# DreamScene-Project/DreamScene

Hardware: AMD Instinct MI355X
Metric: fwd+bwd views/s @1024x1024, 500000 Gaussians (higher is better)
Workload: dtype f32

## Files before the change

### dreamscene_amd/csrc/radix_sort.h

```cpp
#pragma once
#include "gsr_common.h"
#include <type_traits>

namespace {

constexpr int kSortThreads = 256;
constexpr int kItemsLarge = 16;
constexpr int kItemsSmall = 4;
constexpr int kRadixBits = 8;
constexpr int kRadix = 1 << kRadixBits;

template <typename T>
__device__ __forceinline__ T* batch_ptr(T* p, size_t bstride) {
  typedef typename std::conditional<std::is_const<T>::value, const char, char>::type B;
  return p ? reinterpret_cast<T*>(reinterpret_cast<B*>(p) + (size_t)blockIdx.y * bstride) : p;
}
#define GSR_LDS_ORDER() asm volatile("" ::: "memory")

__device__ __forceinline__ uint64_t eff_count(const uint64_t* n_dev, uint64_t cap) {
  if (!n_dev) return cap;
  const uint64_t n = *n_dev;
  return n < cap ? n : cap;
}

// ... 183 lines not shown
    if (is_valid(it)) {
      const uint32_t d = (key[it] >> shift) & (kRadix - 1);
      const uint32_t pos = wh[wave][d] + rank[it];
      keys_out[pos] = key[it];
      vals_out[pos] = val[it];
    }
  }
}

#ifndef GSR_OS_ITEMS_SMALL
#define GSR_OS_ITEMS_SMALL 16
#endif
constexpr int kOsItemsSmall = GSR_OS_ITEMS_SMALL;
constexpr int kOsMaxPasses = 4;
#ifndef GSR_OS_HIST_TILE
#define GSR_OS_HIST_TILE 2048
#endif
constexpr uint32_t kOsHistTile = GSR_OS_HIST_TILE;
constexpr uint32_t kOsTableOff = kOsMaxPasses * kRadix + 16;
constexpr uint32_t kOsSkipFlag = kOsMaxPasses * kRadix + 8;
constexpr uint32_t kOsEarlyN = kOsMaxPasses * kRadix + 10;
constexpr uint64_t kOsMaxN = 1ull << 28;

typedef __attribute__((address_space(1))) uint32_t gsr_gu32;
__device__ __forceinline__ gsr_gu32* gsr_global(uint32_t* p) { return (gsr_gu32*)(uintptr_t)p; }

__host__ __device__ inline uint32_t os_tiles(uint64_t n, int items) {
  const uint64_t t = (uint64_t)kSortThreads * items;
  return (uint32_t)((n + t - 1) / t);
}
__host__ inline size_t os_state_words(uint64_t n, int items) { return (size_t)kOsTableOff + (size_t)kRadix * os_tiles(n, items); }

template <bool DROP>
__global__ void __launch_bounds__(kSortThreads)
k_os_hist(const uint32_t* __restrict__ keys, const uint64_t* __restrict__ n_dev, uint64_t cap, int passes,
          uint32_t* __restrict__ os, size_t bstride, const uint32_t* __restrict__ wrect) {
  keys = batch_ptr(keys, bstride); n_dev = batch_ptr(n_dev, bstride); os = batch_ptr(os, bstride);
  wrect = batch_ptr(wrect, bstride);
  __shared__ uint32_t h[kOsMaxPasses][kRadix];
  __shared__ uint32_t wsum[kSortThreads / 64];
  const int tid = threadIdx.x, lane = tid & 63;
  const uint64_t n = eff_count(n_dev, cap);
  const uint64_t base = (uint64_t)blockIdx.x * kOsHistTile;
  if (base >= n) return;
#pragma unroll
  for (int p = 0; p < kOsMaxPasses; ++p) h[p][tid] = 0;
  __syncthreads();
  constexpr int kPer = kOsHistTile / kSortThreads;
  uint32_t kk[kPer];
  uint32_t weight = 0;
#pragma unroll
  for (int it = 0; it < kPer; ++it) {
    const uint64_t e = base + (uint64_t)(it * kSortThreads + tid);
    kk[it] = e < n ? keys[e] : 0xFFFFFFFFu;
    if (wrect && e < n && (!DROP || kk[it] != 0xFFFFFFFFu)) {
      const uint32_t r = wrect[e];
      weight += (((r >> 16) & 255u) + 1u) * ((r >> 24) + 1u);
    }
  }
  if (wrect) {
#pragma unroll
    for (int o = 32; o > 0; o >>= 1) weight += (uint32_t)__shfl_xor((int)weight, o, 64);
    if (lane == 0) wsum[tid >> 6] = weight;
  }
#pragma unroll
  for (int it = 0; it < kPer; ++it) {
    const uint64_t e = base + (uint64_t)(it * kSortThreads + tid);
    const bool valid = (e < n) && (!DROP || kk[it] != 0xFFFFFFFFu);
    const unsigned long long vm = __ballot(valid);
    if (vm == 0ull) continue;
    const uint32_t k = kk[it];
    if (valid) {
      atomicAdd(&h[0][k & (kRadix - 1)], 1u);
      if (passes > 1) atomicAdd(&h[1][(k >> kRadixBits) & (kRadix - 1)], 1u);
    }
    if (passes > 2) {
      const int first = __ffsll((long long)vm) - 1;
      const uint32_t hi = k >> (2 * kRadixBits), hi0 = (uint32_t)__shfl((int)hi, first, 64);
      if (__ballot(valid && hi != hi0) == 0ull) {
        if (lane == first) {
          atomicAdd(&h[2][hi0 & (kRadix - 1)], (uint32_t)__popcll(vm));
          if (passes > 3) atomicAdd(&h[3][hi0 >> kRadixBits], (uint32_t)__popcll(vm));
        }
      } else if (valid) {
        atomicAdd(&h[2][hi & (kRadix - 1)], 1u);
        if (passes > 3) atomicAdd(&h[3][hi >> kRadixBits], 1u);
      }
    }
  }
  __syncthreads();
  for (int p = 0; p < passes; ++p) {
    const uint32_t c = h[p][tid];
    if (c) atomicAdd(&os[p * kRadix + tid], c);
  }
  if (wrect && tid == 0) {
    const uint64_t w = ((uint64_t)wsum[0] + wsum[1]) + ((uint64_t)wsum[2] + wsum[3]);
    if (w) atomicAdd(reinterpret_cast<unsigned long long*>(os + kOsEarlyN), (unsigned long long)w);
  }
}

#ifndef GSR_OS_WINDOW
#define GSR_OS_WINDOW 16
#endif
constexpr int kOsWindow = GSR_OS_WINDOW;
__device__ __forceinline__ uint32_t os_look_back(gsr_gu32* table, uint32_t tile, int col, uint32_t tagA, uint32_t tagI) {
  uint32_t excl = 0;
  int p = (int)tile - 1;
  for (;;) {
    uint32_t w[kOsWindow];
#pragma unroll
    for (int j = 0; j < kOsWindow; ++j)
      w[j] = (p - j >= 0) ? __hip_atomic_load(table + (size_t)(p - j) * kRadix + col, __ATOMIC_RELAXED, __HIP_MEMORY_SCOPE_AGENT)
                          : 0u;
    bool done = false, stalled = false;
#pragma unroll
    for (int j = 0; j < kOsWindow; ++j) {
      if (done || stalled) continue;
      const uint32_t tag = w[j] & 0xF0000000u;
      if (tag == tagI) { excl += w[j] & 0x0FFFFFFFu; done = true; }
      else if (tag == tagA) { excl += w[j] & 0x0FFFFFFFu; --p; }
      else stalled = true;
    }
    if (done) return excl;
    if (stalled) __builtin_amdgcn_s_sleep(1);
  }
}

#ifdef GSR_OS_TRACE
__device__ unsigned long long* g_os_trace = nullptr;
#define GSR_OS_STAMP(k) do { if (threadIdx.x == 0 && g_os_trace) \
    g_os_trace[(((size_t)pass * 4 + blockIdx.y) * 4096 + blockIdx.x) * 8 + (k)] = wall_clock64(); } while (0)
#else
#define GSR_OS_STAMP(k) do { } while (0)
#endif

template <bool IOTA, int ITEMS, bool DROP>
__global__ void __launch_bounds__(kSortThreads)
k_os_pass(const uint32_t* __restrict__ keys_in, const uint32_t* __restrict__ vals_in, uint32_t* __restrict__ keys_out,
          uint32_t* __restrict__ vals_out, const uint64_t* __restrict__ n_dev, uint64_t cap, int pass,
          uint32_t* __restrict__ os, uint64_t* __restrict__ n_out, size_t bstride, const int may_skip,
          uint64_t* __restrict__ early_out) {
  keys_in = batch_ptr(keys_in, bstride); vals_in = batch_ptr(vals_in, bstride);
  keys_out = batch_ptr(keys_out, bstride); vals_out = batch_ptr(vals_out, bstride);
  n_dev = batch_ptr(n_dev, bstride); os = batch_ptr(os, bstride); n_out = batch_ptr(n_out, bstride);
  constexpr uint32_t T = kSortThreads * ITEMS;
  __shared__ uint32_t wh[4][kRadix];
  __shared__ uint32_t gbase[kRadix];
  __shared__ uint32_t skey[T], sval[T];
  __shared__ uint32_t wtot[4];
  __shared__ uint32_t s_tile, s_ntile;
  const int tid = threadIdx.x, lane = tid & 63, wave = tid >> 6;
  const int shift = pass * kRadixBits;
  const uint64_t n = eff_count(n_dev, cap);
  if constexpr (!DROP) {
    const uint32_t x = os[pass * kRadix + tid];
    if (__syncthreads_or((uint64_t)x == n && n > 0)) {
      if (may_skip) {
        if (blockIdx.x == 0 && tid == 0) os[kOsSkipFlag] = 1u;
        return;
      }
#pragma unroll
      for (int it = 0; it < ITEMS; ++it) {
        const uint64_t e = sort_index<ITEMS>(blockIdx.x, wave, it, lane);
        if (e < n) {
          keys_out[e] = keys_in[e];
          vals_out[e] = IOTA ? (uint32_t)e : vals_in[e];
        }
      }
      return;
    }
  }
  GSR_OS_STAMP(0);
  if (tid == 0) s_tile = atomicAdd(&os[kOsMaxPasses * kRadix + pass], 1u);
#pragma unroll
  for (int w = 0; w < 4; ++w) wh[w][tid] = 0;
  __syncthreads();
  const uint32_t tile = s_tile;
  if (early_out && tile == 0 && tid == 0)
    __hip_atomic_store(early_out + blockIdx.y, *reinterpret_cast<const uint64_t*>(os + kOsEarlyN), __ATOMIC_RELAXED,
                       __HIP_MEMORY_SCOPE_SYSTEM);
  if ((uint64_t)tile * T >= n) return;
  uint32_t dbase;
  {
    const uint32_t x = os[pass * kRadix + tid];
    uint32_t inc = x;
#pragma unroll
    for (int o = 1; o < 64; o <<= 1) {
      const uint32_t t = (uint32_t)__shfl_up((int)inc, o, 64);
      if (lane >= o) inc += t;
    }
    if (lane == 63) wtot[wave] = inc;
    __syncthreads();
    uint32_t woff = 0;
    for (int w = 0; w < wave; ++w) woff += wtot[w];
    dbase = woff + inc - x;
    if (DROP && n_out && tile == 0 && tid == kSortThreads - 1) *n_out = (uint64_t)(woff + inc);
  }
  GSR_OS_STAMP(1);
#ifdef GSR_OS_TRACE
  if (threadIdx.x == 0 && g_os_trace) g_os_trace[(((size_t)pass * 4 + blockIdx.y) * 4096 + blockIdx.x) * 8 + 7] = tile;
#endif
  uint32_t* mywh = wh[wave];
  uint32_t key[ITEMS], val[ITEMS], rank[ITEMS];
  const unsigned long long lt = (1ull << lane) - 1ull;
#pragma unroll
  for (int it = 0; it < ITEMS; ++it) {
    const uint64_t e = sort_index<ITEMS>(tile, wave, it, lane);
    const bool valid = e < n;
    key[it] = valid ? keys_in[e] : 0xFFFFFFFFu;
    val[it] = IOTA ? (uint32_t)e : (valid ? vals_in[e] : 0u);
  }
  const auto is_valid = [&](int it) {
    const uint64_t e = sort_index<ITEMS>(tile, wave, it, lane);
    return (e < n) && (!DROP || key[it] != 0xFFFFFFFFu);
  };
#pragma unroll
  for (int it = 0; it < ITEMS; ++it) {
    const bool valid = is_valid(it);
    const uint32_t d = (key[it] >> shift) & (kRadix - 1);
    const unsigned long long m = match_digit(d, valid);
    const int leader = __ffsll((long long)m) - 1;
    uint32_t old = 0;
    if (valid && lane == leader) {
      old = mywh[d];
      mywh[d] = old + (uint32_t)__popcll(m);
    }
    old = (uint32_t)__shfl((int)old, valid ? leader : lane, 64);
    rank[it] = old + (uint32_t)__popcll(m & lt);
    GSR_LDS_ORDER();
  }
  __syncthreads();
  GSR_OS_STAMP(2);
  uint32_t cnt;
  {
    uint32_t run = 0;
#pragma unroll
    for (int w = 0; w < 4; ++w) {
      const uint32_t c = wh[w][tid];
      wh[w][tid] = run;
      run += c;
    }
    cnt = run;
  }
  gsr_gu32* table = gsr_global(os + kOsTableOff);
  const uint32_t tagA = (uint32_t)(2 * pass + 1) << 28, tagI = (uint32_t)(2 * pass + 2) << 28;
  uint32_t excl = 0;
  if (tile == 0) {
    __hip_atomic_store(table + tid, tagI | cnt, __ATOMIC_RELAXED, __HIP_MEMORY_SCOPE_AGENT);
  } else {
    __hip_atomic_store(table + (size_t)tile * kRadix + tid, tagA | cnt, __ATOMIC_RELAXED, __HIP_MEMORY_SCOPE_AGENT);
    excl = os_look_back(table, tile, tid, tagA, tagI);
    __hip_atomic_store(table + (size_t)tile * kRadix + tid, tagI | (excl + cnt), __ATOMIC_RELAXED, __HIP_MEMORY_SCOPE_AGENT);
  }
  GSR_OS_STAMP(3);
  uint32_t lstart;
  {
    uint32_t inc = cnt;
#pragma unroll
    for (int o = 1; o < 64; o <<= 1) {
      const uint32_t t = (uint32_t)__shfl_up((int)inc, o, 64);
      if (lane >= o) inc += t;
    }
    __syncthreads();
    if (lane == 63) wtot[wave] = inc;
    __syncthreads();
    uint32_t woff = 0;
    for (int w = 0; w < wave; ++w) woff += wtot[w];
    lstart = woff + inc - cnt;
    if (tid == kSortThreads - 1) s_ntile = woff + inc;
  }
#pragma unroll
  for (int w = 0; w < 4; ++w) wh[w][tid] += lstart;
  gbase[tid] = dbase + excl - lstart;
  __syncthreads();
#pragma unroll
  for (int it = 0; it < ITEMS; ++it) {
    if (is_valid(it)) {
      const uint32_t d = (key[it] >> shift) & (kRadix - 1);
      const uint32_t lp = wh[wave][d] + rank[it];
      skey[lp] = key[it];
      sval[lp] = val[it];
    }
  }
  __syncthreads();
  GSR_OS_STAMP(4);
  const uint32_t ntile = s_ntile;
  for (uint32_t i = tid; i < ntile; i += kSortThreads) {
    const uint32_t k = skey[i];
    const uint32_t pos = gbase[(k >> shift) & (kRadix - 1)] + i;
    keys_out[pos] = k;
    vals_out[pos] = sval[i];
  }
  GSR_OS_STAMP(5);
}

__host__ inline size_t align256(size_t x) { return (x + 255) & ~(size_t)255; }

uint32_t sort_blocks(uint64_t n, int items) {
  const uint64_t t = (uint64_t)kSortThreads * items;
  return (uint32_t)((n + t - 1) / t);
}

__host__ inline size_t sort_hist_bytes(uint64_t n, int items_legacy, int items_os) {
  const size_t legacy = (size_t)kRadix * sort_blocks(n, items_legacy) * 4;
  const size_t os = os_state_words(n, items_os) * 4;
  return align256(legacy > os ? legacy : os);
}

template <int ITEMS>
int radix_sort_u32_legacy(uint32_t* k0, uint32_t* v0, uint32_t* k1, uint32_t* v1, const uint64_t* n_dev, uint64_t cap,
                          int bits, bool iota, uint64_t* n_compact, uint32_t* hist, uint32_t* totals, hipStream_t stream,
                          int batch = 1, size_t bstride = 0);

template <int ITEMS, int OS_ITEMS>
int radix_sort_u32(uint32_t* k0, uint32_t* v0, uint32_t* k1, uint32_t* v1, const uint64_t* n_dev, uint64_t cap,
                   int bits, bool iota, uint64_t* n_compact, uint32_t* hist, uint32_t* totals, hipStream_t stream,
                   int batch = 1, size_t bstride = 0, bool state_cleared = false, bool last_pass_may_skip = false,
                   const uint32_t* early_rects = nullptr, uint64_t* early_out = nullptr) {
  const int passes = (bits + kRadixBits - 1) / kRadixBits;
  if (cap >= kOsMaxN || passes > kOsMaxPasses)
    return radix_sort_u32_legacy<ITEMS>(k0, v0, k1, v1, n_dev, cap, bits, iota, n_compact, hist, totals, stream, batch, bstride);
  const uint32_t ntile = os_tiles(cap, OS_ITEMS), nhist = (uint32_t)((cap + kOsHistTile - 1) / kOsHistTile);
  const dim3 grid(ntile, (uint32_t)batch), grid_h(nhist ? nhist : 1, (uint32_t)batch);
  if (!state_cleared &&
      gsr_zero_async(hist, os_state_words(cap, OS_ITEMS) * 4, stream, bstride, (uint32_t)batch) != hipSuccess) return passes & 1;
  const bool drop = iota && n_compact;
  if (!drop) { early_rects = nullptr; early_out = nullptr; }
  if (!early_out) early_rects = nullptr;
  if (drop)
    hipLaunchKernelGGL((k_os_hist<true>), grid_h, dim3(kSortThreads), 0, stream, k0, n_dev, cap, passes, hist, bstride,
                       early_rects);
  else
    hipLaunchKernelGGL((k_os_hist<false>), grid_h, dim3(kSortThreads), 0, stream, k0, n_dev, cap, passes, hist, bstride,
                       (const uint32_t*)nullptr);
  uint32_t *ka = k0, *va = v0, *kb = k1, *vb = v1;
  for (int p = 0; p < passes; ++p) {
    if (p == 0 && drop) {
      hipLaunchKernelGGL((k_os_pass<true, OS_ITEMS, true>), grid, dim3(kSortThreads), 0, stream, ka, va, kb, vb, n_dev, cap, p,
                         hist, n_compact, bstride, 0, early_rects ? early_out : (uint64_t*)nullptr);
      n_dev = n_compact;
    } else if (p == 0 && iota) {
      hipLaunchKernelGGL((k_os_pass<true, OS_ITEMS, false>), grid, dim3(kSortThreads), 0, stream, ka, va, kb, vb, n_dev, cap, p,
                         hist, (uint64_t*)nullptr, bstride, 0, (uint64_t*)nullptr);
    } else {
      hipLaunchKernelGGL((k_os_pass<false, OS_ITEMS, false>), grid, dim3(kSortThreads), 0, stream, ka, va, kb, vb, n_dev, cap, p,
                         hist, (uint64_t*)nullptr, bstride, (last_pass_may_skip && p == passes - 1 && p > 0) ? 1 : 0,
                         (uint64_t*)nullptr);
    }
    uint32_t* t = ka; ka = kb; kb = t;
    t = va; va = vb; vb = t;
  }
  return passes & 1;
}

template <int ITEMS>
int radix_sort_u32_legacy(uint32_t* k0, uint32_t* v0, uint32_t* k1, uint32_t* v1, const uint64_t* n_dev, uint64_t cap,
                   int bits, bool iota, uint64_t* n_compact, uint32_t* hist, uint32_t* totals, hipStream_t stream,
                   int batch, size_t bstride) {
  const uint32_t nblk = sort_blocks(cap, ITEMS);
  const int passes = (bits + kRadixBits - 1) / kRadixBits;
  const dim3 grid(nblk, (uint32_t)batch), grid_scan(kRadix, (uint32_t)batch);
  uint32_t *ka = k0, *va = v0, *kb = k1, *vb = v1;
  for (int p = 0; p < passes; ++p) {
// ... 29 lines not shown
```

### dreamscene_amd/csrc/render_bwd.hip

```cpp
#include "gsr_render.h"

namespace {

struct WorkBwdViews {
  const uint32_t* tile_depth[GSR_MAX_BATCH_VIEWS];
  uint32_t* items[GSR_MAX_BATCH_VIEWS];
  uint32_t items_cap[GSR_MAX_BATCH_VIEWS];
  uint32_t seg_len[GSR_MAX_BATCH_VIEWS];
};

__global__ void __launch_bounds__(1024)
k_work_order_bwd(const uint32_t n_tiles, const WorkBwdViews wv) {
  const uint32_t* __restrict__ tile_depth = wv.tile_depth[blockIdx.x];
  uint32_t* __restrict__ items = wv.items[blockIdx.x];
  const uint32_t items_cap = wv.items_cap[blockIdx.x];
  const uint32_t kb = wv.seg_len[blockIdx.x];
  __shared__ uint32_t cnt[32], cur[32];
  const int tid = threadIdx.x;
  if (tid < 32) cnt[tid] = 0;
  __syncthreads();
  for (uint32_t t = tid; t < n_tiles; t += 1024) {
    const uint32_t d = tile_depth[t];
    if (d == 0) continue;
    const uint32_t full = d / kb, tail = d % kb;
    for (uint32_t sgi = 0; sgi < full; ++sgi) atomicAdd(&cnt[15u - min(15u, (d - kb * sgi - 1u) >> 8)], 1u);
    if (tail) atomicAdd(&cnt[16u + 15u - ((tail - 1u) * 16u) / kb], 1u);
  }
  __syncthreads();
  if (tid == 0) {
    uint32_t run = 0;
    for (int b = 0; b < 32; ++b) { cur[b] = run; run += cnt[b]; }
    items[0] = min(run, items_cap);
  }
  __syncthreads();
  for (uint32_t t = tid; t < n_tiles; t += 1024) {
    const uint32_t d = tile_depth[t];
    if (d == 0) continue;
    const uint32_t full = d / kb, tail = d % kb;
    for (uint32_t sgi = 0; sgi < full; ++sgi) {
      const uint32_t i = atomicAdd(&cur[15u - min(15u, (d - kb * sgi - 1u) >> 8)], 1u);
      if (i < items_cap) { items[2 + 2 * i] = t; items[3 + 2 * i] = sgi; }
    }
    if (tail) {
      const uint32_t i = atomicAdd(&cur[16u + 15u - ((tail - 1u) * 16u) / kb], 1u);
      if (i < items_cap) { items[2 + 2 * i] = t; items[3 + 2 * i] = full; }
    }
  }
}

__device__ __forceinline__ float add_swap32(float a, float b) {
  const auto r = __builtin_amdgcn_permlane32_swap(__float_as_uint(a), __float_as_uint(b), false, false);
  return __uint_as_float(r[0]) + __uint_as_float(r[1]);
}
__device__ __forceinline__ float add_swap16(float a, float b) {
  const auto r = __builtin_amdgcn_permlane16_swap(__float_as_uint(a), __float_as_uint(b), false, false);
  return __uint_as_float(r[0]) + __uint_as_float(r[1]);
}
__device__ __forceinline__ float reduce10(const float v[10]) {
  float p0, p1, p2, p3, p4, q0, q1, q2;
  asm("s_nop 1\n\t"
      "v_add_f32_dpp %0, %8, %8 row_ror:8 row_mask:0xf bank_mask:0x3\n\t"
      "v_add_f32_dpp %0, %9, %9 row_ror:8 row_mask:0xf bank_mask:0xc\n\t"
      "v_add_f32_dpp %1, %10, %10 row_ror:8 row_mask:0xf bank_mask:0x3\n\t"
      "v_add_f32_dpp %1, %11, %11 row_ror:8 row_mask:0xf bank_mask:0xc\n\t"
      "v_add_f32_dpp %2, %12, %12 row_ror:8 row_mask:0xf bank_mask:0x3\n\t"
      "v_add_f32_dpp %2, %13, %13 row_ror:8 row_mask:0xf bank_mask:0xc\n\t"
      "v_add_f32_dpp %3, %14, %14 row_ror:8 row_mask:0xf bank_mask:0x3\n\t"
      "v_add_f32_dpp %3, %15, %15 row_ror:8 row_mask:0xf bank_mask:0xc\n\t"
      "v_add_f32_dpp %4, %16, %16 row_ror:8 row_mask:0xf bank_mask:0x3\n\t"
      "v_add_f32_dpp %4, %17, %17 row_ror:8 row_mask:0xf bank_mask:0xc\n\t"
      "s_nop 1\n\t"
      "v_add_f32_dpp %5, %0, %0 row_half_mirror row_mask:0xf bank_mask:0x5\n\t"
      "v_add_f32_dpp %5, %1, %1 row_half_mirror row_mask:0xf bank_mask:0xa\n\t"
      "v_add_f32_dpp %6, %2, %2 row_half_mirror row_mask:0xf bank_mask:0x5\n\t"
      "v_add_f32_dpp %6, %3, %3 row_half_mirror row_mask:0xf bank_mask:0xa\n\t"
      "v_add_f32_dpp %7, %4, %4 row_half_mirror row_mask:0xf bank_mask:0xf"
      : "=&v"(p0), "=&v"(p1), "=&v"(p2), "=&v"(p3), "=&v"(p4), "=&v"(q0), "=&v"(q1), "=&v"(q2)
      : "v"(v[0]), "v"(v[1]), "v"(v[2]), "v"(v[3]), "v"(v[4]), "v"(v[5]), "v"(v[6]), "v"(v[7]), "v"(v[8]), "v"(v[9]));
  const float r0 = add_swap32(q0, q1);
  float R = add_swap16(r0, q2);
  asm("s_nop 1\n\t"
      "v_add_f32_dpp %0, %0, %0 quad_perm:[2,3,0,1] row_mask:0xf bank_mask:0xf\n\t"
      "s_nop 1\n\t"
      "v_add_f32_dpp %0, %0, %0 quad_perm:[1,0,3,2] row_mask:0xf bank_mask:0xf"
      : "+v"(R));
  return R;
}

template <int KB>
__device__ __forceinline__ void
render_bwd_body(const uint32_t item, const int W, const int H, const uint32_t* __restrict__ items, const uint32_t* __restrict__ tile_depth,
             const float* __restrict__ ckpt,
             const uint32_t* __restrict__ ranges, const uint32_t* __restrict__ point_list,
             const float4* __restrict__ splat, const float* __restrict__ bg, const float* __restrict__ color,
             const float* __restrict__ depth_alpha, const float* __restrict__ final_T,
             const uint32_t* __restrict__ n_contrib, const float* __restrict__ dL_dcolor,
             const float* __restrict__ dL_dda, float* __restrict__ partials, unsigned long long* __restrict__ reach) {
  __shared__ float4 s0[KB], s1[KB], s2[KB];
  __shared__ uint32_t sid[KB], smask[KB];
  __shared__ unsigned long long hitw[KB / 64];
  const int gx = (W + GSR_TILE - 1) / GSR_TILE;
  const int tid = threadIdx.x, wave = tid >> 6, lane = tid & 63;
  if (item >= items[0]) return;
 {
  const int tile = (int)items[2 + 2 * item];
  const uint32_t seg = items[3 + 2 * item];
  const uint32_t depth = tile_depth[tile];
  const uint32_t lo = seg * KB, hi = min(lo + (uint32_t)KB, depth);
  const int n = (int)(hi - lo);

  const TilePix p = tile_pixel(tile, gx, W, H);
  const int tile_x0 = p.bx - (wave & 1) * 8, tile_y0 = p.by - (wave >> 1) * 8;
  const float pxf = (float)p.px, pyf = (float)p.py;
  const uint32_t r0 = ranges[2 * tile];
  const size_t pix = (size_t)p.py * W + p.px, HW = (size_t)H * W;

  const float zref = reinterpret_cast<const float*>(splat + 3 * (size_t)point_list[r0 + (hi - 1u)] + 1)[2];
  {
    float4 n0 = make_float4(0, 0, 0, 0), n1 = n0, n2 = make_float4(0, 0, -1.f, -1.f);
    uint32_t nid = 0;
    if (tid < n) {
      nid = point_list[r0 + (hi - 1u - (uint32_t)tid)];
      const float4* r = splat + 3 * (size_t)nid;
      n0 = r[0]; n1 = r[1]; n2 = r[2];
    }
    if (tid < KB) {
      s0[tid] = stage_row0(n0);
      s1[tid] = stage_row1(n1, zref);
      s2[tid] = n2;
      sid[tid] = nid;
      smask[tid] = (tid < n) ? block_mask_t<8>(n0, n1, n2, tile_x0, tile_y0) : 0u;
    }
    if (tid < KB / 64) hitw[tid] = 0ull;
  }

  const float Tf = p.inside ? final_T[pix] : 0.f;
  const uint32_t last = p.inside ? n_contrib[pix] : 0u;
  float gC0 = 0.f, gC1 = 0.f, gC2 = 0.f, gD = 0.f, gA = 0.f;
  if (p.inside) {
    gC0 = dL_dcolor[pix]; gC1 = dL_dcolor[HW + pix]; gC2 = dL_dcolor[2 * HW + pix];
    gD = dL_dda[pix]; gA = dL_dda[HW + pix];
  }
  const float bg0 = bg[0], bg1 = bg[1], bg2 = bg[2];
  const float bg_dot = (bg0 * gC0 + bg1 * gC1) + bg2 * gC2;

  float T = Tf;
  float R = 0.f, A = 0.f;
  if (last > hi) {
    const float* ck = ckpt_row<KB>(ckpt, r0 + hi, p.py, tile_y0, p.px, tile_x0);
    const float Tc = ck[0];
    const float inv = 1.0f / Tc;
    T = Tc;
    const float rc0 = ((color[pix] - Tf * bg0) - ck[256]) * inv;
    const float rc1 = ((color[HW + pix] - Tf * bg1) - ck[512]) * inv;
    const float rc2 = ((color[2 * HW + pix] - Tf * bg2) - ck[768]) * inv;
    const float rec_z = (depth_alpha[pix] - ck[1024]) * inv;
    const float rec_a = (depth_alpha[HW + pix] - ck[1280]) * inv;
    R = rc0 * gC0 + rc1 * gC1 + rc2 * gC2 + (rec_z - zref * rec_a) * gD;
    A = rec_a;
  }
  const float cshift = zref * gD + gA;

  const int b2 = (lane >> 2) & 1, b3 = (lane >> 3) & 1, b4 = (lane >> 4) & 1, b5 = (lane >> 5) & 1;
  const int comp = b4 ? 8 + 2 * b5 + b3 : (b3 | (b2 << 1) | (b5 << 2));
  const bool commit = ((lane & 3) == 0) && !(b4 && b2);
  __syncthreads();

  for (int k = 0; k < KB / 64; ++k) {
    if (k * 64 >= n) break;
    unsigned long long bits = __ballot((smask[k * 64 + lane] >> wave) & 1u);
    unsigned long long hitk = 0ull;
    while (bits) {
      const int jb = __builtin_ctzll(bits);
      const int j = k * 64 + jb;
      bits &= bits - 1ull;
      const uint32_t pos = hi - 1u - (uint32_t)j;
      const unsigned long long livem = __builtin_amdgcn_ballot_w64(pos < last);
      if (livem == 0ull) continue;
      const float4 a = s0[j];
      const float4 b = s1[j];
      const float dx = a.x - pxf, dy = a.y - pyf;
      const float power = gsr_power(a.z, a.w, b.x, dx, dy);
      const float G = gsr_exp(power);
      const float alpha = fminf(GSR_ALPHA_MAX, gsr_mul(b.y, G));
      const unsigned long long hitm = livem & __builtin_amdgcn_ballot_w64(power <= 0.0f) &
                                      __builtin_amdgcn_ballot_w64(alpha >= GSR_ALPHA_MIN);
      if (hitm == 0ull) continue;
      hitk |= 1ull << jb;
      const bool hit = __builtin_amdgcn_inverse_ballot_w64(hitm);
      float qv = 0.f, wv = 0.f, gdl = 0.f;
      if (hit) {
        const float4 c = s2[j];
        const float inv = __builtin_amdgcn_rcpf(1.0f - alpha);
        T = T * inv;
// ... 97 lines not shown
```

### dreamscene_amd/csrc/render_fwd.hip

```cpp
#include "gsr_render.h"

namespace {

template <int CTRL>
__device__ __forceinline__ int gsr_dpp_i(int v) {
  return __builtin_amdgcn_update_dpp(0, v, CTRL, 0xF, 0xF, true);
}
__device__ __forceinline__ float fold_slots(float x) { x += gsr_dpp<0x124>(x); return x + gsr_dpp<0x128>(x); }

__device__ __forceinline__ void gather_splat(const uint32_t* point_list, const float4* splat, uint32_t pos, uint32_t& nid,
                                             float4& n0, float4& n1, float4& n2) {
  nid = point_list[pos];
  const float4* r = splat + 3 * (size_t)nid;
  n0 = r[0]; n1 = r[1]; n2 = r[2];
}

__device__ __forceinline__ void store_pixel(size_t pix, size_t HW, float T, uint32_t last, float c0, float c1, float c2,
                                            float depth, float alpha, const float* bg, float* out_color, float* out_da,
                                            float* final_T, uint32_t* n_contrib) {
  final_T[pix] = T;
  n_contrib[pix] = last;
  out_color[pix] = c0 + T * bg[0]; out_color[HW + pix] = c1 + T * bg[1]; out_color[2 * HW + pix] = c2 + T * bg[2];
  out_da[pix] = depth; out_da[HW + pix] = alpha;
}

struct WorkFwdViews {
  const uint32_t* ranges[GSR_MAX_BATCH_VIEWS];
  uint32_t* tile_depth[GSR_MAX_BATCH_VIEWS];
  uint32_t* work[GSR_MAX_BATCH_VIEWS];
  uint32_t* stats_host[GSR_MAX_BATCH_VIEWS];
};

#ifndef GSR_ORDER_FRAC_BITS
#define GSR_ORDER_FRAC_BITS 2
#endif
constexpr int kOrderFrac = GSR_ORDER_FRAC_BITS;
constexpr int kOrderClasses = 2 + (32 << kOrderFrac);
__device__ __forceinline__ uint32_t order_class(uint32_t len) {
  if (len == 0u) return 0u;
  const int msb = 31 - __clz(len);
  if constexpr (kOrderFrac == 0) return (uint32_t)msb + 1u;
  const uint32_t frac = (msb >= kOrderFrac ? (len >> (msb - kOrderFrac)) : (len << (kOrderFrac - msb))) & ((1u << kOrderFrac) - 1u);
  return 1u + ((uint32_t)msb << kOrderFrac) + frac;
}
__global__ void __launch_bounds__(1024)
k_work_order_fwd(const uint32_t n_tiles, const WorkFwdViews wv) {
  const uint32_t* __restrict__ ranges = wv.ranges[blockIdx.x];
  uint32_t* __restrict__ tile_depth = wv.tile_depth[blockIdx.x];
  uint32_t* __restrict__ work = wv.work[blockIdx.x];
  uint32_t* __restrict__ stats_host = wv.stats_host[blockIdx.x];
  __shared__ uint32_t cnt[kOrderClasses], cur[kOrderClasses];
  const int tid = threadIdx.x;
  if (tid < kOrderClasses) cnt[tid] = 0;
  __syncthreads();
  for (uint32_t t = tid; t < n_tiles; t += 1024) {
    const uint32_t len = ranges[2 * t + 1] - ranges[2 * t];
    atomicAdd(&cnt[order_class(len)], 1u);
    tile_depth[t] = 0;
  }
  __syncthreads();
  if (tid == 0) {
    uint32_t run = 0;
    for (int b = kOrderClasses - 1; b >= 0; --b) { cur[b] = run; run += cnt[b]; }
    work[n_tiles] = n_tiles - cnt[0];
    if (stats_host) *stats_host = n_tiles - cnt[0];
  }
  __syncthreads();
  for (uint32_t t = tid; t < n_tiles; t += 1024) {
    const uint32_t len = ranges[2 * t + 1] - ranges[2 * t];
    work[atomicAdd(&cur[order_class(len)], 1u)] = t;
  }
}

template <bool SCORE, int PAD = 0>
struct Stage {
  float4 s0[2][kBatch + PAD], s1[2][kBatch + PAD], s2[2][kBatch + PAD];
  uint32_t sid[SCORE ? 2 : 1][SCORE ? kBatch : 1];
  uint32_t cnt[SCORE ? 2 : 1][SCORE ? kBatch : 1];
};

template <bool SCORE, int KB>
__device__ __forceinline__ void
render_fwd_body(const uint32_t item, const int W, const int H, const uint32_t* __restrict__ work, float* __restrict__ ckpt,
             const uint32_t* __restrict__ ranges,
             const uint32_t* __restrict__ point_list, const float4* __restrict__ splat, const float* __restrict__ bg,
             float* __restrict__ out_color, float* __restrict__ out_da, float* __restrict__ final_T,
             uint32_t* __restrict__ n_contrib, uint32_t* __restrict__ tile_depth, float* __restrict__ score,
             const int score_mode) {
  __shared__ Stage<SCORE, 1> st;
  __shared__ uint16_t cand[4][kBatch + 16];
  if (threadIdx.x < 2) {
    st.s0[threadIdx.x][kBatch] = make_float4(0.f, 0.f, 0.f, 0.f);
    st.s1[threadIdx.x][kBatch] = make_float4(0.f, 0.f, 0.f, 0.f);
    st.s2[threadIdx.x][kBatch] = make_float4(0.f, 0.f, 0.f, 0.f);
  }
  if constexpr (SCORE) { st.cnt[0][threadIdx.x] = 0u; st.cnt[1][threadIdx.x] = 0u; }
  auto flush_counts = [&](const int b) {
    if constexpr (SCORE) {
      const uint32_t c = st.cnt[b][threadIdx.x];
      if (c) {
        atomicAdd(reinterpret_cast<uint32_t*>(score) + st.sid[b][threadIdx.x], c);
        st.cnt[b][threadIdx.x] = 0u;
      }
    }
  };
  const int gx = (W + GSR_TILE - 1) / GSR_TILE;
  const int tid = threadIdx.x, wave = tid >> 6, lane = tid & 63;
  const int slot = (lane >> 2) & 3, pcol = lane & 3, prow = lane >> 4;
  const float bg0 = bg[0], bg1 = bg[1], bg2 = bg[2];
  {
    const uint32_t tile = work[item >> 2];
    const int quarter = (int)(item & 3u);
    const int ty = (int)tile / gx, tx = (int)tile - ty * gx;
    const int q_x0 = tx * GSR_TILE + (quarter & 1) * 8, q_y0 = ty * GSR_TILE + (quarter >> 1) * 8;
    const int px = q_x0 + (wave & 1) * 4 + pcol, py = q_y0 + (wave >> 1) * 4 + prow;
    const bool inside = (px < W) && (py < H);
    const float pxf = (float)px, pyf = (float)py;
    const uint32_t r0 = ranges[2 * tile], r1 = ranges[2 * tile + 1];
    if (r0 == r1) {
      if (quarter == 0) {
        const int ex = tx * GSR_TILE + (tid & 15), ey = ty * GSR_TILE + (tid >> 4);
        if (ex < W && ey < H) {
          const size_t pix = (size_t)ey * W + ex, HW = (size_t)H * W;
          final_T[pix] = 1.0f;
          n_contrib[pix] = 0u;
          out_color[pix] = bg0; out_color[HW + pix] = bg1; out_color[2 * HW + pix] = bg2;
          out_da[pix] = 0.f; out_da[HW + pix] = 0.f;
        }
      }
      return;
    }

    unsigned long long donem = __builtin_amdgcn_ballot_w64(!inside);
    float T = 1.0f, C0 = 0.f, C1 = 0.f, C2 = 0.f, Dp = 0.f, Wt = 0.f;
    uint32_t last = 0;

    uint32_t nid = 0;
    float4 n0 = make_float4(0, 0, 0, 0), n1 = n0, n2 = n0;
    if (r0 + tid < r1) gather_splat(point_list, splat, r0 + tid, nid, n0, n1, n2);
    int buf = 0;
    for (uint32_t base = r0; base < r1; base += kBatch, buf ^= 1) {
      const int n = (int)min((uint32_t)kBatch, r1 - base);
      st.s0[buf][tid] = stage_row0(n0);
      st.s1[buf][tid] = stage_row1(n1);
      st.s2[buf][tid] = make_float4(n2.x, n2.y, n2.z,
                                    __uint_as_float((tid < n) ? block_mask_t<4>(n0, n1, n2, q_x0, q_y0) : 0u));
      if constexpr (SCORE) st.sid[buf][tid] = nid;
      const int n_done = __syncthreads_count(__builtin_amdgcn_inverse_ballot_w64(donem));
      if (score_mode != 1 && base != r0) flush_counts(buf ^ 1);
      if (n_done == 256) break;
      auto checkpoint = [&](const uint32_t pos) {
        if (ckpt == nullptr) return;
        const float f0 = fold_slots(C0), f1 = fold_slots(C1), f2 = fold_slots(C2), f3 = fold_slots(Dp), f4 = fold_slots(Wt);
        if (slot == 0 && inside) {
          float* ck = ckpt_row<KB>(ckpt, pos, py, ty * GSR_TILE, px, tx * GSR_TILE);
          ck[0] = T; ck[256] = f0; ck[512] = f1; ck[768] = f2; ck[1024] = f3; ck[1280] = f4;
        }
      };
      if (base != r0) checkpoint(base);
      if (base + kBatch + tid < r1) gather_splat(point_list, splat, base + kBatch + tid, nid, n0, n1, n2);
      int cnt = 0;
      int cut_at[3] = {-1, -1, -1};
#pragma unroll
      for (int k = 0; k < kBatch / 64; ++k) {
        if (k * 64 >= n) break;
        const bool m = (stage_mask(st.s2[buf][k * 64 + lane]) >> wave) & 1u;
        const unsigned long long bal = __builtin_amdgcn_ballot_w64(m);
        if (m) cand[wave][cnt + (int)__builtin_amdgcn_mbcnt_hi((uint32_t)(bal >> 32), __builtin_amdgcn_mbcnt_lo((uint32_t)bal, 0u))] = (uint8_t)(k * 64 + lane);
        cnt += (int)__popcll(bal);
        if constexpr (KB < kBatch) {
          if (((k + 1) * 64) % KB == 0 && k + 1 < kBatch / 64 && (k + 1) * 64 < n) {
            const int pad = (-cnt) & 3;
            if (lane < pad) cand[wave][cnt + lane] = (uint16_t)kBatch;
            cnt += pad;
            cut_at[(k + 1) * 64 / KB - 1] = cnt;
          }
        }
      }
      if (lane < 3) cand[wave][cnt + lane] = (uint16_t)kBatch;
      __builtin_amdgcn_fence(__ATOMIC_ACQ_REL, "wavefront");
      __builtin_amdgcn_wave_barrier();
      {
        for (int i = 0;; i += 4) {
          if (donem == ~0ull) break;
          if constexpr (KB < kBatch) {
#pragma unroll
            for (int c = 0; c < kBatch / KB - 1; ++c)
              if (i == cut_at[c]) checkpoint(base + (uint32_t)((c + 1) * KB));
          }
          if (i >= cnt) break;
          const int j = (int)cand[wave][i + slot];
          const float4 a = st.s0[buf][j];
          const float4 b = st.s1[buf][j];
          const float2 c = *reinterpret_cast<const float2*>(&st.s2[buf][j]);
          const float dx = a.x - pxf, dy = a.y - pyf;
          const float power = gsr_power(a.z, a.w, b.x, dx, dy);
          const float alpha = fminf(GSR_ALPHA_MAX, gsr_mul(b.y, gsr_exp(power)));
          const unsigned long long gm = ~donem & __builtin_amdgcn_ballot_w64(power <= 0.0f) &
                                        __builtin_amdgcn_ballot_w64(alpha >= GSR_ALPHA_MIN);
          const bool g = __builtin_amdgcn_inverse_ballot_w64(gm);
          const float fgate = g ? gsr_sub(1.0f, alpha) : 1.0f;
          float test_T = gsr_mul(T, fgate);
          asm("s_nop 1\n\t"
              "v_mul_f32_dpp %0, %0, %1 row_shr:4 row_mask:0xf bank_mask:0xe\n\t"
              "s_nop 1\n\t"
              "v_mul_f32_dpp %0, %0, %1 row_shr:4 row_mask:0xf bank_mask:0xc\n\t"
              "s_nop 1\n\t"
              "v_mul_f32_dpp %0, %0, %1 row_shr:4 row_mask:0xf bank_mask:0x8"
              : "+v"(test_T) : "v"(fgate));
          float w_all = alpha * T;
          asm("s_nop 1\n\t"
              "v_mul_f32_dpp %0, %1, %2 row_shr:4 row_mask:0xf bank_mask:0xe"
              : "+v"(w_all) : "v"(test_T), "v"(alpha));
          const unsigned long long stopm = __builtin_amdgcn_ballot_w64(test_T < GSR_T_MIN);
          const bool hit = __builtin_amdgcn_inverse_ballot_w64(gm & ~stopm);
          const float w = hit ? w_all : 0.0f;
          C0 = fmaf(b.w, w, C0); C1 = fmaf(c.x, w, C1); C2 = fmaf(c.y, w, C2);
          Dp = fmaf(b.z, w, Dp);
          Wt += w;
          last = hit ? ((base - r0) + (uint32_t)j + 1u) : last;
          if constexpr (SCORE) {
            const unsigned long long hm = __ballot(hit) & (0x000F000F000F000Full << (4 * slot));
            if (score_mode != 1) {
// ... 235 lines not shown
```

Baseline: 5055.

## Prefetch sort tile keys early, batch bucket atomics, parallelize work-order scans

The onesweep radix pass now loads its keys and values using blockIdx.x before the histogram-skip check and tile atomic. It reuses them when the dynamically assigned tile matches blockIdx.x, so the global load latency overlaps the skip check and the prefix scan. The backward work-order kernel groups consecutive segments that fall in the same depth bucket into one atomic, and replaces the serial 32-entry scan with a wave shuffle scan. The forward work-order kernel aggregates empty-tile counts per wave with ballot and scans the class histogram in parallel. The costs are extra register pressure in the sort kernel and wasted loads when the tile differs from blockIdx.x.

Measured after the change: 5033. No clear change (-0.4%).

```diff
diff --git a/dreamscene_amd/csrc/radix_sort.h b/dreamscene_amd/csrc/radix_sort.h
--- a/dreamscene_amd/csrc/radix_sort.h
+++ b/dreamscene_amd/csrc/radix_sort.h
@@ -359,8 +359,17 @@
   const int tid = threadIdx.x, lane = tid & 63, wave = tid >> 6;
   const int shift = pass * kRadixBits;
   const uint64_t n = eff_count(n_dev, cap);
+  const uint32_t hist_x = os[pass * kRadix + tid];
+  uint32_t key[ITEMS], val[ITEMS];
+#pragma unroll
+  for (int it = 0; it < ITEMS; ++it) {
+    const uint64_t e = sort_index<ITEMS>(blockIdx.x, wave, it, lane);
+    const bool valid = e < n;
+    key[it] = valid ? keys_in[e] : 0xFFFFFFFFu;
+    val[it] = IOTA ? (uint32_t)e : (valid ? vals_in[e] : 0u);
+  }
   if constexpr (!DROP) {
-    const uint32_t x = os[pass * kRadix + tid];
+    const uint32_t x = hist_x;
     if (__syncthreads_or((uint64_t)x == n && n > 0)) {
       if (may_skip) {
         if (blockIdx.x == 0 && tid == 0) os[kOsSkipFlag] = 1u;
@@ -389,7 +398,7 @@
   if ((uint64_t)tile * T >= n) return;
   uint32_t dbase;
   {
-    const uint32_t x = os[pass * kRadix + tid];
+    const uint32_t x = hist_x;
     uint32_t inc = x;
 #pragma unroll
     for (int o = 1; o < 64; o <<= 1) {
@@ -408,14 +417,16 @@
   if (threadIdx.x == 0 && g_os_trace) g_os_trace[(((size_t)pass * 4 + blockIdx.y) * 4096 + blockIdx.x) * 8 + 7] = tile;
 #endif
   uint32_t* mywh = wh[wave];
-  uint32_t key[ITEMS], val[ITEMS], rank[ITEMS];
+  uint32_t rank[ITEMS];
   const unsigned long long lt = (1ull << lane) - 1ull;
-#pragma unroll
-  for (int it = 0; it < ITEMS; ++it) {
-    const uint64_t e = sort_index<ITEMS>(tile, wave, it, lane);
-    const bool valid = e < n;
-    key[it] = valid ? keys_in[e] : 0xFFFFFFFFu;
-    val[it] = IOTA ? (uint32_t)e : (valid ? vals_in[e] : 0u);
+  if (tile != blockIdx.x) {
+#pragma unroll
+    for (int it = 0; it < ITEMS; ++it) {
+      const uint64_t e = sort_index<ITEMS>(tile, wave, it, lane);
+      const bool valid = e < n;
+      key[it] = valid ? keys_in[e] : 0xFFFFFFFFu;
+      val[it] = IOTA ? (uint32_t)e : (valid ? vals_in[e] : 0u);
+    }
   }
   const auto is_valid = [&](int it) {
     const uint64_t e = sort_index<ITEMS>(tile, wave, it, lane);
diff --git a/dreamscene_amd/csrc/render_bwd.hip b/dreamscene_amd/csrc/render_bwd.hip
--- a/dreamscene_amd/csrc/render_bwd.hip
+++ b/dreamscene_amd/csrc/render_bwd.hip
@@ -17,29 +17,48 @@
   const uint32_t kb = wv.seg_len[blockIdx.x];
   __shared__ uint32_t cnt[32], cur[32];
   const int tid = threadIdx.x;
+  const auto seg_run = [kb](uint32_t d, uint32_t full, uint32_t s, uint32_t& bucket) {
+    const uint32_t q = min(15u, (d - kb * s - 1u) >> 8);
+    bucket = 15u - q;
+    return min(full, (d - 1u - (q << 8)) / kb + 1u);
+  };
   if (tid < 32) cnt[tid] = 0;
   __syncthreads();
   for (uint32_t t = tid; t < n_tiles; t += 1024) {
     const uint32_t d = tile_depth[t];
     if (d == 0) continue;
     const uint32_t full = d / kb, tail = d % kb;
-    for (uint32_t sgi = 0; sgi < full; ++sgi) atomicAdd(&cnt[15u - min(15u, (d - kb * sgi - 1u) >> 8)], 1u);
+    for (uint32_t s = 0; s < full;) {
+      uint32_t bucket;
+      const uint32_t e = seg_run(d, full, s, bucket);
+      atomicAdd(&cnt[bucket], e - s);
+      s = e;
+    }
     if (tail) atomicAdd(&cnt[16u + 15u - ((tail - 1u) * 16u) / kb], 1u);
   }
   __syncthreads();
-  if (tid == 0) {
-    uint32_t run = 0;
-    for (int b = 0; b < 32; ++b) { cur[b] = run; run += cnt[b]; }
-    items[0] = min(run, items_cap);
+  if (tid < 64) {
+    const uint32_t x = tid < 32 ? cnt[tid] : 0u;
+    uint32_t inc = x;
+#pragma unroll
+    for (int o = 1; o < 32; o <<= 1) {
+      const uint32_t u = (uint32_t)__shfl_up((int)inc, o, 64);
+      if (tid >= o) inc += u;
+    }
+    if (tid < 32) cur[tid] = inc - x;
+    if (tid == 31) items[0] = min(inc, items_cap);
   }
   __syncthreads();
   for (uint32_t t = tid; t < n_tiles; t += 1024) {
     const uint32_t d = tile_depth[t];
     if (d == 0) continue;
     const uint32_t full = d / kb, tail = d % kb;
-    for (uint32_t sgi = 0; sgi < full; ++sgi) {
-      const uint32_t i = atomicAdd(&cur[15u - min(15u, (d - kb * sgi - 1u) >> 8)], 1u);
-      if (i < items_cap) { items[2 + 2 * i] = t; items[3 + 2 * i] = sgi; }
+    for (uint32_t s = 0; s < full;) {
+      uint32_t bucket;
+      const uint32_t e = seg_run(d, full, s, bucket);
+      uint32_t i = atomicAdd(&cur[bucket], e - s);
+      for (; s < e; ++s, ++i)
+        if (i < items_cap) { items[2 + 2 * i] = t; items[3 + 2 * i] = s; }
     }
     if (tail) {
       const uint32_t i = atomicAdd(&cur[16u + 15u - ((tail - 1u) * 16u) / kb], 1u);
diff --git a/dreamscene_amd/csrc/render_fwd.hip b/dreamscene_amd/csrc/render_fwd.hip
--- a/dreamscene_amd/csrc/render_fwd.hip
+++ b/dreamscene_amd/csrc/render_fwd.hip
@@ -50,25 +50,57 @@
   uint32_t* __restrict__ work = wv.work[blockIdx.x];
   uint32_t* __restrict__ stats_host = wv.stats_host[blockIdx.x];
   __shared__ uint32_t cnt[kOrderClasses], cur[kOrderClasses];
-  const int tid = threadIdx.x;
+  constexpr int kScanWaves = (kOrderClasses + 63) / 64;
+  static_assert(kOrderClasses <= 1024, "one thread per class");
+  __shared__ uint32_t wtot[kScanWaves];
+  const int tid = threadIdx.x, lane = tid & 63, wave = tid >> 6;
+  const unsigned long long lt = (1ull << lane) - 1ull;
   if (tid < kOrderClasses) cnt[tid] = 0;
   __syncthreads();
-  for (uint32_t t = tid; t < n_tiles; t += 1024) {
-    const uint32_t len = ranges[2 * t + 1] - ranges[2 * t];
-    atomicAdd(&cnt[order_class(len)], 1u);
-    tile_depth[t] = 0;
+  for (uint32_t t0 = 0; t0 < n_tiles; t0 += 1024) {
+    const uint32_t t = t0 + (uint32_t)tid;
+    const bool in = t < n_tiles;
+    const uint32_t cls = in ? order_class(ranges[2 * t + 1] - ranges[2 * t]) : 1u;
+    const unsigned long long empty = __ballot(in && cls == 0u);
+    if (in && cls != 0u) atomicAdd(&cnt[cls], 1u);
+    if (lane == 0 && empty) atomicAdd(&cnt[0], (uint32_t)__popcll(empty));
+    if (in) tile_depth[t] = 0;
   }
   __syncthreads();
-  if (tid == 0) {
-    uint32_t run = 0;
-    for (int b = kOrderClasses - 1; b >= 0; --b) { cur[b] = run; run += cnt[b]; }
-    work[n_tiles] = n_tiles - cnt[0];
-    if (stats_host) *stats_host = n_tiles - cnt[0];
+  {
+    const int b = kOrderClasses - 1 - tid;
+    const uint32_t x = tid < kOrderClasses ? cnt[b] : 0u;
+    uint32_t inc = x;
+#pragma unroll
+    for (int o = 1; o < 64; o <<= 1) {
+      const uint32_t u = (uint32_t)__shfl_up((int)inc, o, 64);
+      if (lane >= o) inc += u;
+    }
+    if (lane == 63 && wave < kScanWaves) wtot[wave] = inc;
+    __syncthreads();
+    if (tid < kOrderClasses) {
+      uint32_t woff = 0;
+      for (int w = 0; w < wave; ++w) woff += wtot[w];
+      cur[b] = woff + inc - x;
+    }
+    if (tid == 0) {
+      work[n_tiles] = n_tiles - cnt[0];
+      if (stats_host) *stats_host = n_tiles - cnt[0];
+    }
   }
   __syncthreads();
-  for (uint32_t t = tid; t < n_tiles; t += 1024) {
-    const uint32_t len = ranges[2 * t + 1] - ranges[2 * t];
-    work[atomicAdd(&cur[order_class(len)], 1u)] = t;
+  for (uint32_t t0 = 0; t0 < n_tiles; t0 += 1024) {
+    const uint32_t t = t0 + (uint32_t)tid;
+    const bool in = t < n_tiles;
+    const uint32_t cls = in ? order_class(ranges[2 * t + 1] - ranges[2 * t]) : 1u;
+    const unsigned long long empty = __ballot(in && cls == 0u);
+    uint32_t base = 0;
+    if (lane == 0 && empty) base = atomicAdd(&cur[0], (uint32_t)__popcll(empty));
+    base = (uint32_t)__builtin_amdgcn_readfirstlane((int)base);
+    if (in) {
+      const uint32_t at = cls != 0u ? atomicAdd(&cur[cls], 1u) : base + (uint32_t)__popcll(empty & lt);
+      work[at] = t;
+    }
   }
 }
 
```
